# google/ffn

Hardware: NVIDIA H100
Metric: fov_steps_per_sec (higher is better)
Workload: dtype f16

## Files before the change

ffn_b200/_lib.py:

```python

from __future__ import annotations

import ctypes as C
import os

import numpy as np

HERE = os.path.dirname(os.path.abspath(__file__))
LIB_PATH = os.path.join(HERE, 'libffn_b200.so')

COMPUTE_FP16_TC = 0
COMPUTE_FP32 = 1
COMPUTE_FP16X2_TC = 2
IMAGE_U8 = 0
IMAGE_F32 = 1
ARRAY_SEED = 0
ARRAY_SEGMENTATION = 1
ARRAY_QPROB = 2
ARRAY_IMAGE = 3
MASK_MOVEMENT = 0
MASK_SEED = 1
SEED_POLICY_KINDS = {'peaks_2d': 0, 'fill_empty': 1, 'max_peaks': 2}

EXPORTS = [
    'ffn_last_error', 'ffn_engine_create', 'ffn_engine_destroy', 'ffn_engine_set_compute_mode', 'ffn_engine_set_chains', 'ffn_engine_set_grid',
    'ffn_engine_info', 'ffn_engine_profile', 'ffn_engine_trace', 'ffn_predict', 'ffn_canvas_create', 'ffn_canvas_destroy',
    'ffn_canvas_set_mask', 'ffn_canvas_segment_at', 'ffn_canvas_segment_all',
    'ffn_canvas_update_at', 'ffn_canvas_init_seed', 'ffn_canvas_read', 'ffn_canvas_write',
    'ffn_canvas_policy_state_size', 'ffn_canvas_policy_state_get', 'ffn_canvas_policy_state_set',
    'ffn_canvas_set_resume', 'ffn_canvas_trace', 'ffn_canvas_seed_peaks', 'ffn_canvas_seed_policy', 'ffn_canvas_set_max_id', 'ffn_canvas_get_counters', 'ffn_canvas_spec_stats', 'ffn_canvas_device_ptr',
    'ffn_canvas_add_id_offset', 'ffn_decision_points', 'ffn_reseg_eval', 'ffn_selftest_wgmma',
]


class ModelDesc(C.Structure):
  _fields_ = [('fov_zyx', C.c_int32 * 3), ('deltas_zyx', C.c_int32 * 3), ('depth', C.c_int32),
              ('features', C.c_int32)]


class Options(C.Structure):
  _fields_ = [('init_activation', C.c_float), ('pad_value', C.c_float),
              ('move_threshold', C.c_float), ('segment_threshold', C.c_float),
              ('disco_seed_threshold', C.c_float), ('policy_score_threshold', C.c_double),
              ('min_boundary_dist_zyx', C.c_int32 * 3), ('min_segment_size', C.c_int32)]


class SegStats(C.Structure):
  _fields_ = [('iters', C.c_int64), ('min_pos', C.c_int32 * 3), ('max_pos', C.c_int32 * 3),
              ('seed_got_too_weak', C.c_int32), ('queue_len', C.c_int32), ('finished', C.c_int32),
              ('reserved', C.c_int32)]


class Origin(C.Structure):
  _fields_ = [('id', C.c_int32), ('start_zyx', C.c_int32 * 3), ('iters', C.c_int64),
              ('walltime_sec', C.c_double)]


class Overlap(C.Structure):
  _fields_ = [('id', C.c_int32), ('other_id', C.c_int32), ('count', C.c_int64)]
# ... 32 lines not shown


_lib = None


def build_if_needed():
  from . import build as _build
  return _build.build()


def load() -> C.CDLL:
  global _lib
  if _lib is not None:
    return _lib
  if not os.path.exists(LIB_PATH):
    try:
      build_if_needed()
    except Exception as e:
      raise ImportError(
          'libffn_b200.so is missing and could not be built (%s). The FFN engine has no CPU '
          'fallback.' % e) from e
  lib = C.CDLL(LIB_PATH)
  p = C.c_void_p
  i32p = C.POINTER(C.c_int32)
  lib.ffn_last_error.restype = C.c_char_p
  lib.ffn_last_error.argtypes = []
  lib.ffn_engine_create.argtypes = [C.c_int, C.POINTER(ModelDesc), C.POINTER(C.c_void_p),
                                    C.POINTER(C.c_void_p), C.c_int, C.POINTER(p)]
  lib.ffn_engine_destroy.argtypes = [p]
  lib.ffn_engine_destroy.restype = None
  lib.ffn_engine_set_compute_mode.argtypes = [p, C.c_int]
  lib.ffn_engine_set_grid.argtypes = [p, C.c_int]
  lib.ffn_engine_set_chains.argtypes = [p, C.c_int]
  lib.ffn_engine_info.argtypes = [p, C.POINTER(C.c_int64)]
  lib.ffn_engine_profile.argtypes = [p, C.POINTER(C.c_int64), C.c_int]
  lib.ffn_engine_trace.argtypes = [p, C.POINTER(C.c_int64), C.c_int64, C.c_int]
  lib.ffn_predict.argtypes = [p, p, p, C.c_int, p]
  lib.ffn_canvas_create.argtypes = [p, p, C.c_int, i32p, C.c_float, C.c_float, C.POINTER(Options),
                                    C.c_int, C.POINTER(p)]
  lib.ffn_canvas_destroy.argtypes = [p]
  lib.ffn_canvas_destroy.restype = None
  lib.ffn_canvas_set_mask.argtypes = [p, C.c_int, p]
  lib.ffn_canvas_segment_at.argtypes = [p, i32p, C.c_int, C.c_int64, C.POINTER(SegStats)]
  lib.ffn_canvas_segment_all.argtypes = [p, p, C.c_int64, p, C.c_int64, C.POINTER(C.c_int64), p,
                                         C.c_int64, C.POINTER(C.c_int64), C.POINTER(Counters)]
  lib.ffn_canvas_update_at.argtypes = [p, i32p, p]
  lib.ffn_canvas_init_seed.argtypes = [p, i32p]
  lib.ffn_canvas_read.argtypes = [p, C.c_int, i32p, i32p, p]
  lib.ffn_canvas_write.argtypes = [p, C.c_int, i32p, i32p, p]
  lib.ffn_canvas_policy_state_size.argtypes = [p, C.POINTER(C.c_int64), C.POINTER(C.c_int64)]
  lib.ffn_canvas_policy_state_get.argtypes = [p, p, p, i32p]
  lib.ffn_canvas_policy_state_set.argtypes = [p, p, C.c_int64, p, C.c_int64, i32p]
  lib.ffn_canvas_set_resume.argtypes = [p, C.c_int64, i32p, i32p]
  lib.ffn_canvas_trace.argtypes = [p, C.c_int64, p, C.POINTER(C.c_int64)]
  lib.ffn_canvas_seed_peaks.argtypes = [p, C.POINTER(C.c_float), p, p, C.c_int64, C.POINTER(C.c_int64)]
  lib.ffn_canvas_seed_policy.argtypes = [p, C.POINTER(SeedPolicyDesc), p, p, C.c_int64, C.POINTER(C.c_int64)]
  lib.ffn_canvas_set_max_id.argtypes = [p, C.c_int64]
  lib.ffn_canvas_get_counters.argtypes = [p, C.POINTER(Counters)]
  lib.ffn_canvas_spec_stats.argtypes = [p, C.POINTER(C.c_int64)]
  lib.ffn_canvas_device_ptr.argtypes = [p, C.c_int, C.POINTER(p), C.POINTER(C.c_int64)]
  lib.ffn_canvas_add_id_offset.argtypes = [p, C.c_int32]
  lib.ffn_decision_points.argtypes = [C.c_int, C.POINTER(DecisionPointDesc), p, p, C.c_int64, C.POINTER(C.c_int64)]
  lib.ffn_reseg_eval.argtypes = [C.c_int, C.POINTER(ResegEvalDesc), p, p, p, p, p, p, C.c_int64, C.POINTER(C.c_int64)]
  lib.ffn_selftest_wgmma.argtypes = [C.c_int, C.POINTER(C.c_double), C.c_int]
  for name in EXPORTS:
    if name not in ('ffn_last_error', 'ffn_engine_destroy', 'ffn_canvas_destroy'):
# ... 17 lines not shown
```

ffn_b200/csrc/device_types.cuh:

```cuda
#pragma once

#include <cuda.h>
#include <cuda_fp16.h>
#include <cuda_runtime.h>
#include <stdint.h>

#include "../../include/ffn_b200.h"

namespace ffn {

constexpr int kThreads = 320;
constexpr int kLoadWarp = 8;
constexpr int kSigWarp = 9;
constexpr int kActStages = 3;
constexpr int kTileM = 128;
constexpr int kTileOut = 126;
constexpr int kStackN = 96;
constexpr int kFeat = 32;
constexpr int kAccRegs = 64 * kStackN / 128;
constexpr int kMaxConv = 32;
constexpr int kMaxChains = 4;
constexpr int kBufsPerChain = 6;
constexpr int kMaxBufs = kMaxChains * kBufsPerChain;
constexpr int kSplitShift = 10;
constexpr int kMaxTilesPerCta = 0xFFFF / kTileOut;
static_assert(kMaxChains >= 1 && kMaxChains <= 5, "chains");

struct Geom {
  int fz, fy, fx;
  int mz, my, mx;
  int dz, dy, dx;
  int nconv;
  int xp, pp;
  int nr;
  int nt;
  int halo;
  int guard;
  int rows_alloc;
  int V;
  float inv_pp, inv_xp;
};

struct Weights {
  const __half* w16;
  const __half* w16x2;
  const float* w32;
  const float* bias;
  const float* w_lom;
  float b_lom;
};

constexpr int kTraceEvents = 8, kTraceTiles = 2048, kTraceCta = 1;

constexpr unsigned kRowValid = 1, kRowX0 = 2, kRowXLast = 4;

struct Workspace {
  const uint8_t* row_flags;
  __half* act0_l;
  __half* act_l[2];
  float4* act0_f;
  float4* act_f[2];
  float4* res;
  unsigned* bar;
  int* abort_flag;
  long long* prof;
};

struct CanvasDev {
  const void* image;
  int image_is_u8;
  float mean, stddev;
  int* seg;
  uint8_t* qprob;
  const uint8_t* mask;
  const uint8_t* seed_mask;
  int sz, sy, sx;
  FfnOptions opt;
  float policy_th_f32;
  int q_cap;
  int traj_cap;
  int* trace;
  int trace_cap;
  int lat_dim[3], lat_off[3];
};

struct CanvasState;
struct ObjDev {
  float* seed;
  float* q_score;
  int* q_pos;
  unsigned* lattice;
  int* traj;
  CanvasState* st;
};

struct ChainDev {
  __half* act0_h;
  __half* act_h[2];
  float* seed_raw[2];
  float* logits;
  unsigned* count;
  unsigned* bar;
  float* res;
};

enum Phase : int {
  PH_IDLE = 0,
  PH_START_SEGMENT,
  PH_AFTER_CLEAR,
  PH_AFTER_STEP,
  PH_POP,
  PH_NEXT_SEED,
  PH_AFTER_COUNT,
  PH_AFTER_WRITE,
  PH_SEGMENT_DONE,
  PH_ALL_DONE,
  PH_FORCE_STEP,
  PH_FINISHED,
  PH_FREE,
};

struct CanvasState {
  int phase;
  int q_head, q_tail;
  unsigned epoch;
  int start[3];
  int cur[3];
  int have_cur;
  int min_pos[3], max_pos[3];
  long long iters;
  int dirty_lo[3], dirty_hi[3];
  long long seed_index;
  int spec;
  int fin_round;
  int reset_seed;
// ... 143 lines not shown
```

ffn_b200/csrc/engine.cu:

```cuda
#include <algorithm>
#include <cmath>
#include <cstdio>
#include <cstdlib>
#include <cstring>
#include <memory>
#include <string>
#include <vector>

#include "device_types.cuh"
#define FFN_KNS plain
#define FFN_PROFILE 0
#include "flood_kernel.cuh"
#undef FFN_KNS
#undef FFN_PROFILE
#define FFN_KNS profiled
#define FFN_PROFILE 1
#include "flood_kernel.cuh"
#undef FFN_KNS
#undef FFN_PROFILE
#include "seed_kernels.cuh"
#include "decision_kernels.cuh"
#include "reseg_kernels.cuh"
#include "selftest.cuh"

// ... 164 lines not shown
}

int launch(FfnEngine* e, FfnCanvas* c, int nchains, const Job& job) {
  KParams p{};
  p.g = e->g;
  p.w = e->w;
  p.ws = e->ws;
  if (!e->profiling) p.ws.prof = nullptr;
  if (c) p.cv = c->cv;
  p.nchains = nchains;
  for (int k = 0; k < kMaxChains; ++k) p.ch[k] = e->cws[k];
  for (int b = 0; b < kMaxBufs; ++b) {
    if (c && b < c->nbufs_alloc) p.ob[b] = c->ob[b];
    p.ob[b].st = c ? c->d_state + b : e->d_dummy_state + b;
  }
  p.sched = c ? c->d_sched : e->d_dummy_sched;
  p.ctl = e->d_ctl;
  p.round_flag = e->d_round_flag;
  p.snap = c ? c->d_snap : nullptr;
  std::memcpy(p.tmap, e->tmap, sizeof(p.tmap));
  p.use_tmap = e->use_tmap;
  p.job = job;
  {
    const char* env = std::getenv("FFN_B200_WATCHDOG_S");
    const long long secs = env ? std::atoll(env) : 60;
    p.job.watchdog_ns = (secs > 0 ? secs : 60) * 1000000000ll;
  }
  p.compute_mode = e->compute_mode;
  CUDA_OK(cudaMemsetAsync(e->ws.bar, 0, sizeof(unsigned), cudaStreamPerThread));
  CUDA_OK(cudaMemsetAsync(e->ws.abort_flag, 0, sizeof(int), cudaStreamPerThread));
  CUDA_OK(cudaMemsetAsync(e->d_ctl, 0, sizeof(Ctl), cudaStreamPerThread));
  CUDA_OK(cudaMemsetAsync(e->d_round_flag, 0, sizeof(unsigned), cudaStreamPerThread));
  for (int k = 0; k < kMaxChains; ++k) CUDA_OK(cudaMemsetAsync(e->cws[k].bar, 0, sizeof(unsigned), cudaStreamPerThread));
  void* args[] = {&p};
  CUDA_OK(cudaEventRecord(e->ev0, cudaStreamPerThread));
  CUDA_OK(cudaLaunchCooperativeKernel(flood_kernel(e), dim3(e->grid), dim3(kThreads), args, (size_t)e->smem_bytes,
                                      cudaStreamPerThread));
  CUDA_OK(cudaEventRecord(e->ev1, cudaStreamPerThread));
  CUDA_OK(cudaStreamSynchronize(cudaStreamPerThread));
  float ms = 0.f;
  CUDA_OK(cudaEventElapsedTime(&ms, e->ev0, e->ev1));
  e->last_kernel_seconds = ms * 1e-3;
  e->launches++;
  int abort_flag = 0;
  CUDA_OK(cudaMemcpy(&abort_flag, e->ws.abort_flag, sizeof(int), cudaMemcpyDeviceToHost));
  if (abort_flag != 0)
    return fail("device-side wait timed out (abort code " + std::to_string(abort_flag) +
                "): 1 = grid barrier, 2 = mbarrier, 3 = chain barrier, 4 = round flag, 5 = launch exceeded 60 s");
  return 0;
}

int pull_state(FfnCanvas* c) {
  CUDA_OK(cudaMemcpy(&c->h_state, c->d_state, sizeof(CanvasState), cudaMemcpyDeviceToHost));
  return 0;
}
int push_state(FfnCanvas* c) {
  CUDA_OK(cudaMemcpy(c->d_state, &c->h_state, sizeof(CanvasState), cudaMemcpyHostToDevice));
  return 0;
}

int alloc_buf(FfnCanvas* c, int k) {
  ObjDev& ch = c->ob[k];
  if (k > 0) {
    if (dev_alloc(&ch.seed, c->nvox, false)) return 1;
    fill_f32_kernel<<<c->eng->sm_count * 8, 256, 0, cudaStreamPerThread>>>(ch.seed, c->nvox, NAN);
    CUDA_OK(cudaGetLastError());
// ... 58 lines not shown

void pack_weights(const Geom& g, const float* const* w, std::vector<__half>& w16, std::vector<__half>& w16x2,
                  std::vector<float>& w32) {
  const int nconv = g.nconv;
  w16.assign(w16_layer_offset_halfs(nconv), __float2half(0.f));
  w16x2.assign(2 * w16_layer_offset_halfs(nconv), __float2half(0.f));
  w32.assign(w32_layer_offset_floats(nconv), 0.f);
  for (int l = 0; l < nconv; ++l) {
    const int cin = l == 0 ? 2 : 32;
    const int nch = l == 0 ? 2 : 4;
    const int cin_pad = l == 0 ? 4 : 32;
    __half* d16 = w16.data() + w16_layer_offset_halfs(l);
    __half* d16hi = w16x2.data() + 2 * w16_layer_offset_halfs(l);
    __half* d16lo = d16hi + (w16_layer_offset_halfs(l + 1) - w16_layer_offset_halfs(l));
    float* d32 = w32.data() + w32_layer_offset_floats(l);
    for (int tap = 0; tap < 27; ++tap)
      for (int ci = 0; ci < cin; ++ci)
        for (int co = 0; co < 32; ++co) {
          const float v = w[l][((size_t)tap * cin + ci) * 32 + co];
          {
            const int row = tap / 3, n = (tap % 3) * 32 + co;
            const size_t at = (((size_t)row * nch + ci / 8) * 12 + n / 8) * 64 + (n % 8) * 8 + (ci % 8);
            d16[at] = __float2half_rn(v);
            const float vs = v * (float)(1 << kSplitShift);
            const __half h = __float2half_rn(vs);
            d16hi[at] = h;
            d16lo[at] = __float2half_rn(vs - __half2float(h));
          }
          d32[((size_t)tap * cin_pad + ci) * 32 + co] = v;
        }
  }
}

int box_copy(FfnCanvas* c, int which, const int32_t lo[3], const int32_t sz[3], void* host, bool to_host) {
  const CanvasDev& cv = c->cv;
  for (int k = 0; k < 3; ++k) {
    const int dim = k == 0 ? cv.sz : k == 1 ? cv.sy : cv.sx;
    if (lo[k] < 0 || sz[k] <= 0 || lo[k] + sz[k] > dim) return fail("box out of canvas bounds");
  }
  size_t esz = 0;
  char* base = nullptr;
  switch (which) {
    case FFN_ARRAY_SEED: esz = 4; base = reinterpret_cast<char*>(c->ob[0].seed); break;
    case FFN_ARRAY_SEGMENTATION: esz = 4; base = reinterpret_cast<char*>(cv.seg); break;
    case FFN_ARRAY_QPROB:
      if (!cv.qprob) return fail("canvas was created without probability maps");
      esz = 1; base = reinterpret_cast<char*>(cv.qprob); break;
    default: return fail("unknown array id");
  }
  cudaMemcpy3DParms prm{};
  cudaPitchedPtr dev = make_cudaPitchedPtr(base, (size_t)cv.sx * esz, (size_t)cv.sx * esz, cv.sy);
  cudaPitchedPtr hst = make_cudaPitchedPtr(host, (size_t)sz[2] * esz, (size_t)sz[2] * esz, sz[1]);
  prm.extent = make_cudaExtent((size_t)sz[2] * esz, sz[1], sz[0]);
  if (to_host) {
    prm.srcPtr = dev;
    prm.srcPos = make_cudaPos((size_t)lo[2] * esz, lo[1], lo[0]);
    prm.dstPtr = hst;
    prm.kind = cudaMemcpyDeviceToHost;
  } else {
    prm.dstPtr = dev;
    prm.dstPos = make_cudaPos((size_t)lo[2] * esz, lo[1], lo[0]);
    prm.srcPtr = hst;
    prm.kind = cudaMemcpyHostToDevice;
  }
  CUDA_OK(cudaMemcpy3D(&prm));
  return 0;
// ... 69 lines not shown
  CUDA_OK(cudaMemcpy(d_wlom, weights_dhwio[g.nconv], 32 * sizeof(float), cudaMemcpyHostToDevice));
  e->w.w16 = d_w16;
  e->w.w32 = d_w32;
  e->w.bias = d_bias;
  e->w.w_lom = d_wlom;
  e->w.b_lom = biases[g.nconv][0];
  e->owned = {d_w16, d_w16x2, d_w32, d_bias, d_wlom};

  Workspace& ws = e->ws;
  const size_t ra = (size_t)g.rows_alloc;
  if (dev_alloc(&ws.act0_l, 2 * ra * 8)) return 1;
  if (dev_alloc(&ws.act_l[0], 4 * ra * 8)) return 1;
  if (dev_alloc(&ws.act_l[1], 4 * ra * 8)) return 1;
  if (dev_alloc(&ws.act0_f, ra)) return 1;
  if (dev_alloc(&ws.act_f[0], 8 * ra)) return 1;
  if (dev_alloc(&ws.act_f[1], 8 * ra)) return 1;
  if (dev_alloc(&ws.res, 8 * ra)) return 1;
  if (dev_alloc(&ws.bar, 1)) return 1;
  if (dev_alloc(&ws.abort_flag, 1)) return 1;
  if (dev_alloc(&ws.prof, 32 + kTraceEvents * kTraceTiles)) return 1;
  for (void* p : std::vector<void*>{ws.act0_l, ws.act_l[0], ws.act_l[1], ws.act0_f, ws.act_f[0], ws.act_f[1], ws.res,
                                    ws.bar, ws.abort_flag, ws.prof})
    e->owned.push_back(p);
  {
    std::vector<uint8_t> flags((size_t)g.nt * 64);
    for (int t = 0; t < g.nt; ++t)
      for (int i = 0; i < 64; ++i) flags[(size_t)t * 64 + i] = row_flags_byte(g, t, i / 8, i % 8);
    uint8_t* d_flags = nullptr;
    if (dev_alloc(&d_flags, flags.size())) return 1;
    e->owned.push_back(d_flags);
    CUDA_OK(cudaMemcpy(d_flags, flags.data(), flags.size(), cudaMemcpyHostToDevice));
    ws.row_flags = d_flags;
  }
  for (int k = 0; k < kMaxChains; ++k) {
    ChainDev& cw = e->cws[k];
    if (dev_alloc(&cw.act0_h, 2 * ra * 8)) return 1;
    if (dev_alloc(&cw.act_h[0], 4 * ra * 8)) return 1;
    if (dev_alloc(&cw.act_h[1], 4 * ra * 8)) return 1;
    if (dev_alloc(&cw.seed_raw[0], (size_t)g.nt * kTileM)) return 1;
    if (dev_alloc(&cw.seed_raw[1], (size_t)g.nt * kTileM)) return 1;
    if (dev_alloc(&cw.logits, (size_t)g.nt * kTileM)) return 1;
    if (dev_alloc(&cw.count, 4)) return 1;
    if (dev_alloc(&cw.bar, 1)) return 1;
    if (dev_alloc(&cw.res, (size_t)g.nt * kTileM * kFeat)) return 1;
    for (void* p : std::vector<void*>{cw.act0_h, cw.act_h[0], cw.act_h[1], cw.seed_raw[0], cw.seed_raw[1], cw.logits,
                                      cw.count, cw.bar, cw.res})
      e->owned.push_back(p);
  }
  {
    typedef CUresult (*EncodeFn)(CUtensorMap*, CUtensorMapDataType, cuuint32_t, void*, const cuuint64_t*, const cuuint64_t*,
                                 const cuuint32_t*, const cuuint32_t*, CUtensorMapInterleave, CUtensorMapSwizzle,
                                 CUtensorMapL2promotion, CUtensorMapFloatOOBfill);
    void* fn = nullptr;
    cudaDriverEntryPointQueryResult qres;
    bool ok = cudaGetDriverEntryPoint("cuTensorMapEncodeTiled", &fn, cudaEnableDefault, &qres) == cudaSuccess && fn &&
              qres == cudaDriverEntryPointSuccess;
    const int seg_rows = kTileOut + 2 * g.halo;
    for (int k = 0; ok && k < kMaxChains; ++k)
      for (int i = 0; ok && i < 3; ++i) {
        const cuuint32_t nch = i == 0 ? 2 : 4;
        void* base = i == 0 ? (void*)e->cws[k].act0_h : (void*)e->cws[k].act_h[i - 1];
        const cuuint64_t dims[4] = {8, (cuuint64_t)(g.rows_alloc - 2 * g.pp), 3, nch};
        const cuuint64_t strides[3] = {16, (cuuint64_t)g.pp * 16, (cuuint64_t)g.rows_alloc * 16};
        const cuuint32_t box[4] = {8, (cuuint32_t)seg_rows, 3, nch};
        const cuuint32_t estr[4] = {1, 1, 1, 1};
        ok = reinterpret_cast<EncodeFn>(fn)(&e->tmap[k][i], CU_TENSOR_MAP_DATA_TYPE_FLOAT16, 4, base, dims, strides, box, estr,
                                            CU_TENSOR_MAP_INTERLEAVE_NONE, CU_TENSOR_MAP_SWIZZLE_NONE,
                                            CU_TENSOR_MAP_L2_PROMOTION_L2_128B, CU_TENSOR_MAP_FLOAT_OOB_FILL_NONE) == CUDA_SUCCESS;
      }
    const char* env = std::getenv("FFN_B200_TMAP");
    e->use_tmap = (ok && env && std::atoi(env) != 0) ? 1 : 0;
  }
  if (dev_alloc(&e->d_ctl, 1)) return 1;
  if (dev_alloc(&e->d_round_flag, 1)) return 1;
  if (dev_alloc(&e->d_dummy_state, kMaxBufs)) return 1;
  if (dev_alloc(&e->d_dummy_sched, 1)) return 1;
  for (void* p : std::vector<void*>{e->d_ctl, e->d_round_flag, e->d_dummy_state, e->d_dummy_sched}) e->owned.push_back(p);
  *out = e.release();
  return 0;
}

void ffn_engine_destroy(FfnEngine* e) {
  if (!e || e->closing) return;
  if (e->live_canvases > 0) {
    e->closing = true;
    return;
  }
  engine_free(e);
}

int ffn_engine_set_grid(FfnEngine* e, int num_ctas) {
  if (!e) return fail("null engine");
  if (num_ctas <= 0) num_ctas = std::min(e->sm_count, e->g.nt);
  if (num_ctas > e->sm_count || num_ctas > e->g.nt) return fail("grid larger than the SM / tile count");
  if ((e->g.nt + num_ctas - 1) / num_ctas > kMaxTilesPerCta)
    return fail("grid too small: at most " + std::to_string(kMaxTilesPerCta) + " tiles per CTA");
  e->grid = num_ctas;
  return 0;
}

int ffn_engine_set_chains(FfnEngine* e, int max_chains) {
  if (!e) return fail("null engine");
  if (max_chains <= 0) max_chains = kMaxChains;
  if (max_chains > kMaxChains) return fail("at most " + std::to_string(kMaxChains) + " chains");
  e->max_chains = max_chains;
  return 0;
}

int ffn_engine_set_compute_mode(FfnEngine* e, int mode) {
  if (!e) return fail("null engine");
  if (mode != FFN_COMPUTE_FP16_TC && mode != FFN_COMPUTE_FP32 && mode != FFN_COMPUTE_FP16X2_TC)
    return fail("unknown compute mode");
  e->compute_mode = mode;
  return 0;
}

int ffn_engine_info(FfnEngine* e, int64_t info[8]) {
  if (!e || !info) return fail("null argument");
  info[0] = e->sm_count;
  info[1] = e->grid;
  info[2] = e->smem_bytes;
  info[3] = e->g.nt;
  info[4] = e->g.nr;
  info[5] = e->g.V;
  info[6] = e->launches;
  info[7] = (int64_t)(e->last_kernel_seconds * 1e9);
  return 0;
}

int ffn_engine_profile(FfnEngine* e, int64_t out[32], int reset) {
// ... 1113 lines not shown
```

ffn_b200/csrc/flood_kernel.cuh:

```cuda

#include <math_constants.h>

#include <utility>

#include "device_types.cuh"
#include "sm90.cuh"

namespace ffn {
namespace FFN_KNS {

struct Ctx {
  const KParams* p;
  int tid, warp, lane, cta, G;
  int t_begin, t_end;
  unsigned bar_target;
  unsigned ev0, ev1, ev2, ev3, ev4;
  unsigned round;
  unsigned long long t_start;
  unsigned char* smem;
  float* s_bias;
  uint64_t* mb_w;
  uint64_t* mb_full;
  uint64_t* mb_empty;
  uint64_t* mb_sig;
  unsigned load_cnt, epi_cnt;
  int* s_misc;
  int* s_round;
  float* s_xchg;
  CanvasState* s_state;
  Sched* s_sched;
  long long* prof;
#if FFN_PROFILE
  unsigned sig_cnt;
#endif
  uint32_t bits;
};

__device__ __forceinline__ uint32_t bit_get(const Ctx& c, int k) { return (c.bits >> k) & 1u; }
__device__ __forceinline__ void bit_flip(Ctx& c, int k) { c.bits ^= 1u << k; }
__device__ __forceinline__ void bit_set(Ctx& c, int k, bool v) { c.bits = (c.bits & ~(1u << k)) | ((v ? 1u : 0u) << k); }

__device__ __forceinline__ unsigned ev_get(const Ctx& c, int k) {
  return k == 0 ? c.ev0 : (k == 1 ? c.ev1 : (k == 2 ? c.ev2 : (k == 3 ? c.ev3 : c.ev4)));
}
__device__ __forceinline__ void ev_add(Ctx& c, int k, unsigned n) {
  if (k == 0) c.ev0 += n;
  else if (k == 1) c.ev1 += n;
  else if (k == 2) c.ev2 += n;
  else if (k == 3) c.ev3 += n;
  else c.ev4 += n;
}
__device__ __forceinline__ CanvasState* chain_state(const Ctx& c, int k) {
  return reinterpret_cast<CanvasState*>(reinterpret_cast<unsigned char*>(c.s_state) + k * kStateSlot);
}

__device__ __forceinline__ void chain_tiles(const Ctx& c, int k, int& tb, int& te) {
  const int nt = c.p->g.nt, base = nt / c.G, extra = nt % c.G;
  const int q = (c.cta + c.G - (k * extra) % c.G) % c.G;
  tb = q * base + min(q, extra);
  te = tb + base + (q < extra ? 1 : 0);
}

__device__ __forceinline__ bool aborted(const Ctx& c) {
  return sm90::ld_volatile_s32(c.p->ws.abort_flag) != 0;
}

#if FFN_PROFILE
__device__ __forceinline__ long long prof_now(const Ctx& c) { return c.prof ? clock64() : 0ll; }
__device__ __forceinline__ void prof_add(const Ctx& c, int slot, long long dt) {
  if (c.prof) c.prof[slot] += dt;
}
__device__ __forceinline__ void trace_ev(const Ctx& c, int ev, unsigned idx) {
  long long* trace = c.p->ws.prof;
  if (trace && c.cta == kTraceCta && idx < (unsigned)kTraceTiles) trace[32 + ev * kTraceTiles + idx] = clock64();
}
#else
__device__ __forceinline__ long long prof_now(const Ctx&) { return 0ll; }
__device__ __forceinline__ void prof_add(const Ctx&, int, long long) {}
__device__ __forceinline__ void trace_ev(const Ctx&, int, unsigned) {}
#endif

__device__ __forceinline__ void mbar_wait(const Ctx& c, uint64_t* bar, uint32_t parity) {
  unsigned spins = 0;
  long long t0 = 0;
  while (!sm90::mbar_try_wait(bar, parity)) {
    if ((++spins & 0x3FF) == 0) {
      if (aborted(c)) return;
      const long long now = clock64();
      if (t0 == 0) t0 = now;
      if (now - t0 > (1ll << 32)) {
        atomicExch(c.p->ws.abort_flag, 2);
        return;
      }
// ... 10 lines not shown
      const long long now = clock64();
      if (tw == 0) tw = now;
      if (now - tw > (1ll << 32)) {
        atomicExch(c.p->ws.abort_flag, code);
        break;
      }
    }
  }
}

__device__ __forceinline__ void grid_barrier(Ctx& c) {
  __syncthreads();
  c.bar_target += c.G;
  if (c.warp == kLoadWarp) {
    if (c.lane == 0) {
      const long long t0 = prof_now(c);
      sm90::red_release_add(c.p->ws.bar, 1u);
      spin_until(c, c.p->ws.bar, c.bar_target, 1);
      prof_add(c, 0, prof_now(c) - t0);
    }
    __syncwarp();
    asm volatile("bar.arrive 4, %0;" ::"n"(kThreads) : "memory");
  } else {
    asm volatile("bar.sync 4, %0;" ::"n"(kThreads) : "memory");
  }
}

__device__ __forceinline__ void chain_arrive_epi(Ctx& c, int k) {
  __syncwarp();
  if (c.lane == 0) sm90::mbar_arrive(&c.mb_sig[k]);
}
__device__ __forceinline__ void chain_signal(Ctx& c, int k, uint32_t parity) {
  mbar_wait(c, &c.mb_sig[k], parity);
  if (c.lane == 0) sm90::red_release_add(c.p->ch[k].bar, 1u);
  __syncwarp();
}
__device__ __forceinline__ void chain_wait(Ctx& c, int k, unsigned events) {
  if (c.lane == 0) {
    const long long t0 = prof_now(c);
    spin_until(c, c.p->ch[k].bar, (unsigned)c.G * (ev_get(c, k) + events), 3);
    prof_add(c, 14, prof_now(c) - t0);
  }
  __syncwarp();
}

__device__ __forceinline__ bool row_to_zyx(const Geom& g, int r, int& z, int& y, int& x) {
  if (r >= g.nr) return false;
  z = (int)(((float)r + 0.5f) * g.inv_pp);
  const int rem = r - z * g.pp;
  y = (int)(((float)rem + 0.5f) * g.inv_xp);
  x = rem - y * g.xp;
  return y < g.fy && x < g.fx;
}

__device__ __forceinline__ bool disco_active(const KParams& p, int k, unsigned parity) {
  if (!(p.cv.opt.disco_seed_threshold >= 0.f)) return false;
  const unsigned cnt = __ldcg(p.ch[k].count + 2 * parity);
  return (double)cnt / (double)p.g.V > (double)p.cv.opt.disco_seed_threshold;
}

__device__ __forceinline__ float merged_row(const KParams& p, int k, unsigned parity, int r, bool disco) {
  float l = __ldcg(p.ch[k].logits + r);
  if (disco) {
    const float o = __ldcg(p.ch[k].seed_raw[parity] + r);
    if (o < 0.f && l > o) l = o;
  }
  return l;
}

__device__ __forceinline__ void stage_fov(Ctx& c, int k, int b, int pz, int py, int px, int batch_idx) {
  const KParams& p = *c.p;
  const Geom& g = p.g;
  const ChainDev& ch = p.ch[k];
  const bool predict = p.job.mode == MODE_PREDICT;
  const unsigned par = c.round & 1u;
// ... 302 lines not shown
}

template <bool X2>
__device__ __forceinline__ int tc_epilogue_any(Ctx& c, int k, int layer, int tile, const EpiBase& e, unsigned flags,
                                               const float (&d)[kAccRegs]) {
  if (layer == c.p->g.nconv - 1) return tc_epilogue<EPI_LAST, X2>(c, k, layer, tile, e, flags, d);
  if (!(layer & 1)) return tc_epilogue<EPI_A, X2>(c, k, layer, tile, e, flags, d);
  if (layer == 1) return tc_epilogue<EPI_B_FIRST, X2>(c, k, layer, tile, e, flags, d);
  return tc_epilogue<EPI_B, X2>(c, k, layer, tile, e, flags, d);
}

__device__ __forceinline__ void publish_counts(Ctx& c, int k, int hit) {
  hit = __reduce_add_sync(0xffffffffu, hit);
  if (c.lane == 0 && hit) atomicAdd(&c.s_misc[k], hit);
  asm volatile("bar.sync 5, 256;" ::: "memory");
  if (c.tid == 0 && c.s_misc[k]) {
    const unsigned packed = (unsigned)c.s_misc[k];
    unsigned* cnt = c.p->ch[k].count + 2 * (c.round & 1u);
    if (packed & 0xffffu) atomicAdd(cnt, packed & 0xffffu);
    if (packed >> 16) atomicAdd(cnt + 1, packed >> 16);
  }
}

__device__ __forceinline__ void layers_pipelined(Ctx& c, unsigned mask) {
  const KParams& p = *c.p;
  const Geom& g = p.g;
  unsigned char* act_smem = c.smem + 2 * 27 * 4 * 512;
  const int seg_rows = kTileOut + 2 * g.halo;
  const int stage_bytes = 3 * 4 * seg_rows * 16;
  const int nconv = g.nconv;
  if (c.tid == 0) prof_add(c, 11, -prof_now(c));

  if (c.warp == kLoadWarp) {
    for (int layer = 0; layer < nconv; ++layer) {
      const int nch = layer == 0 ? 2 : 4;
      const unsigned n0 = c.load_cnt;
      bool weights_pending = true;
      for (int k = 0; k < kMaxChains; ++k) {
        if (!((mask >> k) & 1u)) continue;
        const ChainDev& ch = p.ch[k];
        const __half* in = layer == 0 ? ch.act0_h : ch.act_h[(layer - 1) & 1];
        chain_wait(c, k, (unsigned)layer + 1u);
        if (c.lane == 0) trace_ev(c, 0, c.load_cnt);
        sm90::fence_proxy_async_global();
        int tb, te;
        chain_tiles(c, k, tb, te);
        for (int tile = tb; tile < te; ++tile) {
          const int s = c.load_cnt % kActStages;
          mbar_wait(c, &c.mb_empty[s], ((c.load_cnt / kActStages) & 1u) ^ 1u);
          if (weights_pending && c.load_cnt - n0 == (unsigned)(kActStages - 1)) {
            weights_pending = false;
            if (sm90::elect_one()) tc_issue_weight_load(c, (layer + 1 == nconv) ? 0 : layer + 1);
            __syncwarp();
          }
          const int r0 = tile * kTileOut;
          unsigned char* dst = act_smem + (size_t)s * stage_bytes;
          if (sm90::elect_one()) {
            sm90::mbar_expect_tx(&c.mb_full[s], (uint32_t)(3 * nch * seg_rows * 16));
            if (p.use_tmap) {
              sm90::tma_load_4d(dst, &p.tmap[k][layer == 0 ? 0 : 1 + ((layer - 1) & 1)], 0, g.guard + r0 - g.halo - g.pp, 0, 0,
                                &c.mb_full[s]);
            } else {
              for (int cc = 0; cc < nch; ++cc)
                for (int dzi = 0; dzi < 3; ++dzi)
                  sm90::bulk_g2s(dst + (size_t)(cc * 3 + dzi) * seg_rows * 16,
                                 in + ((size_t)cc * g.rows_alloc + g.guard + r0 + (dzi - 1) * g.pp - g.halo) * 8,
                                 (uint32_t)seg_rows * 16, &c.mb_full[s]);
            }
          }
          __syncwarp();
          if (c.lane == 0) trace_ev(c, 1, c.load_cnt);
          ++c.load_cnt;
        }
      }
      if (weights_pending) {
// ... 1343 lines not shown
  }
}

__device__ __forceinline__ void commit_write(Ctx& c, int b) {
  const KParams& p = *c.p;
  const CanvasState* st = p.ob[b].st;
  int lo[3], hi[3];
  load3(st->box_lo, lo);
  load3(st->box_hi, hi);
  const int nz = hi[0] - lo[0], ny = hi[1] - lo[1], nx = hi[2] - lo[2];
  const long long lines = (long long)nz * ny;
  const int sid = __ldcg(&st->cur_sid);
  for (long long l = (long long)c.cta * (kThreads / 32) + c.warp; l < lines; l += (long long)c.G * (kThreads / 32)) {
    const int z = lo[0] + (int)(l / ny), y = lo[1] + (int)(l % ny);
    const size_t base = cv_index(p.cv, z, y, lo[2]);
    for (int x = c.lane; x < nx; x += 32) {
      const float s = __ldcg(p.ob[b].seed + base + x);
      if (!(s >= p.cv.opt.segment_threshold)) continue;
      if (__ldcg(p.cv.seg + base + x) > 0) continue;
      p.cv.seg[base + x] = sid;
      if (p.cv.qprob) p.cv.qprob[base + x] = quantize_prob(s);
    }
  }
}

template <bool kSplit>
__device__ __forceinline__ void run_layers(Ctx& c, unsigned mask) {
  const KParams& p = *c.p;
  if (!kSplit && p.compute_mode == FFN_COMPUTE_FP16_TC) {
    __syncthreads();
    if (c.tid == 0) {
#pragma unroll
      for (int k = 0; k < kMaxChains; ++k)
        if ((mask >> k) & 1u) sm90::red_release_add(p.ch[k].bar, 1u);
    }
    layers_pipelined(c, mask);
  } else {
    layers_blocking<kSplit>(c);
  }
}

template <bool kSplit>
__global__ void __launch_bounds__(kThreads, 1) ffn_flood_kernel(const __grid_constant__ KParams p) {
  extern __shared__ __align__(1024) unsigned char smem_raw[];
  Ctx c;
  c.p = &p;
  c.tid = threadIdx.x;
  c.warp = __shfl_sync(0xffffffffu, (int)(threadIdx.x >> 5), 0);
  c.lane = threadIdx.x & 31;
  c.cta = blockIdx.x;
  c.G = gridDim.x;
  c.t_begin = (int)(((long long)c.cta * p.g.nt) / c.G);
  c.t_end = (int)(((long long)(c.cta + 1) * p.g.nt) / c.G);
  c.bar_target = 0;
  c.ev0 = c.ev1 = c.ev2 = c.ev3 = c.ev4 = 0;
  c.round = 0;
  c.t_start = sm90::globaltimer_ns();
  c.smem = smem_raw;
  const SmemLayout L = smem_layout(p.g);
  c.s_bias = reinterpret_cast<float*>(smem_raw + L.bias);
  c.mb_w = reinterpret_cast<uint64_t*>(smem_raw + L.bars);
  c.mb_full = c.mb_w + 2;
  c.mb_empty = c.mb_full + kActStages;
  c.mb_sig = c.mb_empty + kActStages;
  c.load_cnt = c.epi_cnt = 0;
  c.s_misc = reinterpret_cast<int*>(smem_raw + L.bars + kOffMisc);
  c.s_round = reinterpret_cast<int*>(smem_raw + L.bars + kOffRound);
// ... 187 lines not shown
```

include/ffn_b200.h:

```cpp
#ifndef FFN_B200_H_
#define FFN_B200_H_

#include <stdint.h>

#ifdef __cplusplus
extern "C" {
#endif

typedef struct FfnEngine FfnEngine;
typedef struct FfnCanvas FfnCanvas;

enum {
  FFN_COMPUTE_FP16_TC = 0,
  FFN_COMPUTE_FP32 = 1,
  FFN_COMPUTE_FP16X2_TC = 2
};

enum { FFN_IMAGE_U8 = 0, FFN_IMAGE_F32 = 1 };

enum { FFN_ARRAY_SEED = 0, FFN_ARRAY_SEGMENTATION = 1, FFN_ARRAY_QPROB = 2, FFN_ARRAY_IMAGE = 3 };

enum { FFN_MASK_MOVEMENT = 0, FFN_MASK_SEED = 1 };

typedef struct {
// ... 34 lines not shown
typedef struct {
  int32_t id;
  int32_t other_id;
  int64_t count;
} FfnOverlap;

typedef struct {
  int64_t inference_calls;
  int64_t segment_at_calls;
  int64_t seeds_examined;
  int64_t skip_threshold;
  int64_t skip_invalid_pos;
  int64_t skip_restricted_pos;
  int64_t seed_got_too_weak;
  int64_t voxels_segmented;
  int64_t voxels_overlapping;
  int64_t invalid_weak;
  int64_t invalid_small;
  int64_t invalid_other;
  int64_t segments;
  int64_t max_id;
  double device_seconds;
  int64_t kernel_launches;
} FfnCounters;

const char* ffn_last_error(void);

int ffn_engine_create(int device, const FfnModelDesc* model, const float* const* weights_dhwio,
                      const float* const* biases, int compute_mode, FfnEngine** out);
void ffn_engine_destroy(FfnEngine* engine);
int ffn_engine_set_compute_mode(FfnEngine* engine, int compute_mode);
int ffn_engine_set_chains(FfnEngine* engine, int max_chains);
int ffn_engine_set_grid(FfnEngine* engine, int num_ctas);
int ffn_engine_info(FfnEngine* engine, int64_t info[8]);

int ffn_engine_profile(FfnEngine* engine, int64_t out[32], int reset);
int ffn_engine_trace(FfnEngine* engine, int64_t* out, int64_t n, int reset);

int ffn_predict(FfnEngine* engine, const float* seed, const float* image, int batch,
                float* logits_out);

int ffn_canvas_create(FfnEngine* engine, const void* image, int image_dtype,
                      const int32_t shape_zyx[3], float image_mean, float image_stddev,
                      const FfnOptions* options, int keep_probability_maps, FfnCanvas** out);
void ffn_canvas_destroy(FfnCanvas* canvas);
int ffn_canvas_set_mask(FfnCanvas* canvas, int which, const uint8_t* mask);

int ffn_canvas_segment_at(FfnCanvas* canvas, const int32_t start_zyx[3], int reset,
                          int64_t max_steps, FfnSegStats* out);

int ffn_canvas_segment_all(FfnCanvas* canvas, const int32_t* seeds_zyx, int64_t n_seeds,
                           FfnOrigin* origins_out, int64_t origins_cap, int64_t* n_origins,
                           FfnOverlap* overlaps_out, int64_t overlaps_cap, int64_t* n_overlaps,
                           FfnCounters* counters_out);

int ffn_canvas_update_at(FfnCanvas* canvas, const int32_t pos_zyx[3], float* pred_out);

int ffn_canvas_init_seed(FfnCanvas* canvas, const int32_t pos_zyx[3]);

int ffn_canvas_read(FfnCanvas* canvas, int which, const int32_t lo_zyx[3],
                    const int32_t size_zyx[3], void* dst);
int ffn_canvas_write(FfnCanvas* canvas, int which, const int32_t lo_zyx[3],
                     const int32_t size_zyx[3], const void* src);

int ffn_canvas_policy_state_size(FfnCanvas* canvas, int64_t* queue_len, int64_t* done_len);
int ffn_canvas_policy_state_get(FfnCanvas* canvas, double* queue_szyx, int32_t* done_zyx,
// ... 81 lines not shown
```

Measured before the change: 6367.

## Replace grid-wide chain barrier with per-CTA progress counters and neighbour waits

Each CTA now publishes its own progress counter per chain, and the load warp waits only on the CTAs whose tile ranges overlap its halo, using a host-computed neighbour table, instead of a barrier counting signals from the whole grid. The aim is to stop a CTA from stalling on slow, unrelated CTAs between conv layers so layers can overlap across the grid. In exchange it adds more polling loads, a neighbour-table upload whenever the grid changes, and a correctness risk if the halo reasoning behind the table is wrong.

```diff
diff --git a/ffn_b200/_lib.py b/ffn_b200/_lib.py
--- a/ffn_b200/_lib.py
+++ b/ffn_b200/_lib.py
@@ -24,7 +24,7 @@
 
 EXPORTS = [
     'ffn_last_error', 'ffn_engine_create', 'ffn_engine_destroy', 'ffn_engine_set_compute_mode', 'ffn_engine_set_chains', 'ffn_engine_set_grid',
-    'ffn_engine_info', 'ffn_engine_profile', 'ffn_engine_trace', 'ffn_predict', 'ffn_canvas_create', 'ffn_canvas_destroy',
+    'ffn_chain_neighbours', 'ffn_engine_info', 'ffn_engine_profile', 'ffn_engine_trace', 'ffn_predict', 'ffn_canvas_create', 'ffn_canvas_destroy',
     'ffn_canvas_set_mask', 'ffn_canvas_segment_at', 'ffn_canvas_segment_all',
     'ffn_canvas_update_at', 'ffn_canvas_init_seed', 'ffn_canvas_read', 'ffn_canvas_write',
     'ffn_canvas_policy_state_size', 'ffn_canvas_policy_state_get', 'ffn_canvas_policy_state_set',
@@ -123,6 +123,7 @@
   lib.ffn_engine_set_compute_mode.argtypes = [p, C.c_int]
   lib.ffn_engine_set_grid.argtypes = [p, C.c_int]
   lib.ffn_engine_set_chains.argtypes = [p, C.c_int]
+  lib.ffn_chain_neighbours.argtypes = [C.POINTER(ModelDesc), C.c_int, C.c_int, i32p, i32p]
   lib.ffn_engine_info.argtypes = [p, C.POINTER(C.c_int64)]
   lib.ffn_engine_profile.argtypes = [p, C.POINTER(C.c_int64), C.c_int]
   lib.ffn_engine_trace.argtypes = [p, C.POINTER(C.c_int64), C.c_int64, C.c_int]
diff --git a/ffn_b200/csrc/device_types.cuh b/ffn_b200/csrc/device_types.cuh
--- a/ffn_b200/csrc/device_types.cuh
+++ b/ffn_b200/csrc/device_types.cuh
@@ -41,6 +41,18 @@
   float inv_pp, inv_xp;
 };
 
+__host__ __device__ inline void chain_tiles(int nt, int G, int k, int cta, int& tb, int& te) {
+  const int base = nt / G, extra = nt % G;
+  const int q = (cta + G - (k * extra) % G) % G;
+  tb = q * base + (q < extra ? q : extra);
+  te = tb + base + (q < extra ? 1 : 0);
+}
+
+constexpr int kMaxNeighbours = 32;
+constexpr int kMaxNeighbourGrid = 255;
+constexpr int kProgStride = 8;
+static_assert(kMaxChains <= 4, "the neighbour table packs 16 bits per chain into 64");
+
 struct Weights {
   const __half* w16;
   const __half* w16x2;
@@ -62,6 +74,7 @@
   float4* act_f[2];
   float4* res;
   unsigned* bar;
+  const uint64_t* nbr;
   int* abort_flag;
   long long* prof;
 };
@@ -101,6 +114,7 @@
   float* logits;
   unsigned* count;
   unsigned* bar;
+  unsigned* prog;
   float* res;
 };
 
diff --git a/ffn_b200/csrc/engine.cu b/ffn_b200/csrc/engine.cu
--- a/ffn_b200/csrc/engine.cu
+++ b/ffn_b200/csrc/engine.cu
@@ -220,6 +220,7 @@
   CUDA_OK(cudaMemsetAsync(e->d_ctl, 0, sizeof(Ctl), cudaStreamPerThread));
   CUDA_OK(cudaMemsetAsync(e->d_round_flag, 0, sizeof(unsigned), cudaStreamPerThread));
   for (int k = 0; k < kMaxChains; ++k) CUDA_OK(cudaMemsetAsync(e->cws[k].bar, 0, sizeof(unsigned), cudaStreamPerThread));
+  CUDA_OK(cudaMemsetAsync(e->cws[0].prog, 0, (size_t)kMaxChains * e->sm_count * kProgStride * sizeof(unsigned), cudaStreamPerThread));
   void* args[] = {&p};
   CUDA_OK(cudaEventRecord(e->ev0, cudaStreamPerThread));
   CUDA_OK(cudaLaunchCooperativeKernel(flood_kernel(e), dim3(e->grid), dim3(kThreads), args, (size_t)e->smem_bytes,
@@ -344,6 +345,48 @@
   }
 }
 
+void chain_neighbours(const Geom& g, int G, int k, int32_t* first, int32_t* count) {
+  const int base = g.nt / G, extra = g.nt % G, rot = (k * extra) % G;
+  auto slot_of = [&](int t) { return t < extra * (base + 1) ? t / (base + 1) : extra + (t - extra * (base + 1)) / base; };
+  std::vector<int> rlo(G), rhi(G);
+  for (int q = 0; q < G; ++q) {
+    int tb, te;
+    ffn::chain_tiles(g.nt, G, k, (q + rot) % G, tb, te);
+    const int lo = tb * kTileOut - g.pp - g.halo, hi = te * kTileOut + g.pp + g.halo;
+    rlo[q] = slot_of(std::max(lo, 0) / kTileOut);
+    rhi[q] = slot_of(std::min((hi - 1) / kTileOut, g.nt - 1));
+  }
+  std::vector<int> lo(G), hi(G);
+  bool whole = false;
+  for (int q = 0; q < G; ++q) {
+    lo[q] = rlo[q];
+    hi[q] = rhi[q];
+    for (int i = 0; i < G; ++i)
+      if (rlo[i] <= q && q <= rhi[i]) {
+        lo[q] = std::min(lo[q], i);
+        hi[q] = std::max(hi[q], i);
+      }
+    whole |= hi[q] - lo[q] + 1 > kMaxNeighbours;
+  }
+  for (int q = 0; q < G; ++q) {
+    const int cta = (q + rot) % G;
+    first[cta] = whole ? 0 : (lo[q] + rot) % G;
+    count[cta] = whole ? G : hi[q] - lo[q] + 1;
+  }
+}
+
+int upload_neighbours(FfnEngine* e) {
+  const int G = e->grid;
+  std::vector<uint64_t> packed(G, 0);
+  std::vector<int32_t> first(G), count(G);
+  for (int k = 0; k < kMaxChains; ++k) {
+    chain_neighbours(e->g, G, k, first.data(), count.data());
+    for (int j = 0; j < G; ++j) packed[j] |= (uint64_t)((uint32_t)first[j] | (uint32_t)count[j] << 8) << (16 * k);
+  }
+  CUDA_OK(cudaMemcpy(const_cast<uint64_t*>(e->ws.nbr), packed.data(), G * sizeof(uint64_t), cudaMemcpyHostToDevice));
+  return 0;
+}
+
 int box_copy(FfnCanvas* c, int which, const int32_t lo[3], const int32_t sz[3], void* host, bool to_host) {
   const CanvasDev& cv = c->cv;
   for (int k = 0; k < 3; ++k) {
@@ -479,6 +522,17 @@
     CUDA_OK(cudaMemcpy(d_flags, flags.data(), flags.size(), cudaMemcpyHostToDevice));
     ws.row_flags = d_flags;
   }
+  if (e->sm_count > kMaxNeighbourGrid) return fail("more SMs than the neighbour table of the chain waits holds");
+  {
+    uint64_t* d_nbr = nullptr;
+    unsigned* d_prog = nullptr;
+    if (dev_alloc(&d_nbr, (size_t)e->sm_count)) return 1;
+    if (dev_alloc(&d_prog, (size_t)kMaxChains * e->sm_count * kProgStride)) return 1;
+    e->owned.push_back(d_nbr);
+    e->owned.push_back(d_prog);
+    ws.nbr = d_nbr;
+    for (int k = 0; k < kMaxChains; ++k) e->cws[k].prog = d_prog + (size_t)k * e->sm_count * kProgStride;
+  }
   for (int k = 0; k < kMaxChains; ++k) {
     ChainDev& cw = e->cws[k];
     if (dev_alloc(&cw.act0_h, 2 * ra * 8)) return 1;
@@ -523,6 +577,7 @@
   if (dev_alloc(&e->d_dummy_state, kMaxBufs)) return 1;
   if (dev_alloc(&e->d_dummy_sched, 1)) return 1;
   for (void* p : std::vector<void*>{e->d_ctl, e->d_round_flag, e->d_dummy_state, e->d_dummy_sched}) e->owned.push_back(p);
+  if (upload_neighbours(e.get())) return 1;
   *out = e.release();
   return 0;
 }
@@ -542,7 +597,19 @@
   if (num_ctas > e->sm_count || num_ctas > e->g.nt) return fail("grid larger than the SM / tile count");
   if ((e->g.nt + num_ctas - 1) / num_ctas > kMaxTilesPerCta)
     return fail("grid too small: at most " + std::to_string(kMaxTilesPerCta) + " tiles per CTA");
+  if (set_device(e)) return 1;
   e->grid = num_ctas;
+  return upload_neighbours(e);
+}
+
+int ffn_chain_neighbours(const FfnModelDesc* model, int num_ctas, int chain, int32_t* first, int32_t* count) {
+  if (!model || !first || !count) return fail("null argument");
+  for (int k = 0; k < 3; ++k)
+    if (model->fov_zyx[k] < 3 || model->fov_zyx[k] % 2 == 0) return fail("fov sizes must be odd and >= 3");
+  const Geom g = make_geom(*model);
+  if (num_ctas < 1 || num_ctas > g.nt || num_ctas > kMaxNeighbourGrid) return fail("grid outside [1, min(tiles, 255)]");
+  if (chain < 0 || chain >= kMaxChains) return fail("bad chain index");
+  chain_neighbours(g, num_ctas, chain, first, count);
   return 0;
 }
 
diff --git a/ffn_b200/csrc/flood_kernel.cuh b/ffn_b200/csrc/flood_kernel.cuh
--- a/ffn_b200/csrc/flood_kernel.cuh
+++ b/ffn_b200/csrc/flood_kernel.cuh
@@ -55,10 +55,7 @@
 }
 
 __device__ __forceinline__ void chain_tiles(const Ctx& c, int k, int& tb, int& te) {
-  const int nt = c.p->g.nt, base = nt / c.G, extra = nt % c.G;
-  const int q = (c.cta + c.G - (k * extra) % c.G) % c.G;
-  tb = q * base + min(q, extra);
-  te = tb + base + (q < extra ? 1 : 0);
+  ffn::chain_tiles(c.p->g.nt, c.G, k, c.cta, tb, te);
 }
 
 __device__ __forceinline__ bool aborted(const Ctx& c) {
@@ -135,15 +132,43 @@
 }
 __device__ __forceinline__ void chain_signal(Ctx& c, int k, uint32_t parity) {
   mbar_wait(c, &c.mb_sig[k], parity);
-  if (c.lane == 0) sm90::red_release_add(c.p->ch[k].bar, 1u);
+  if (c.lane == 0) sm90::red_release_add(c.p->ch[k].prog + c.cta * kProgStride, 1u);
   __syncwarp();
 }
-__device__ __forceinline__ void chain_wait(Ctx& c, int k, unsigned events) {
+__device__ __forceinline__ void chain_wait_staged(Ctx& c, int k) {
   if (c.lane == 0) {
     const long long t0 = prof_now(c);
-    spin_until(c, c.p->ch[k].bar, (unsigned)c.G * (ev_get(c, k) + events), 3);
+    spin_until(c, c.p->ch[k].bar, (unsigned)c.G * (ev_get(c, k) / (unsigned)c.p->g.nconv + 1u), 3);
     prof_add(c, 14, prof_now(c) - t0);
   }
+  __syncwarp();
+}
+__device__ __forceinline__ void chain_wait_neighbours(Ctx& c, int k, unsigned events, uint32_t nb) {
+  const long long t0 = prof_now(c);
+  const int first = (int)(nb & 0xFFu), count = (int)((nb >> 8) & 0xFFu);
+  const unsigned target = ev_get(c, k) + events;
+  const unsigned* prog = c.p->ch[k].prog;
+  unsigned spins = 0;
+  long long tw = 0;
+  for (;;) {
+    bool done = true;
+    for (int i = c.lane; i < count; i += 32) {
+      const int j = first + i < c.G ? first + i : first + i - c.G;
+      done &= (int)(sm90::ld_acquire_u32(prog + j * kProgStride) - target) >= 0;
+    }
+    if (__all_sync(0xffffffffu, done)) break;
+    if ((++spins & 0xFF) == 0) {
+      const bool stop = aborted(c);
+      const long long now = clock64();
+      if (tw == 0) tw = now;
+      const bool late = now - tw > (1ll << 32);
+      if (__any_sync(0xffffffffu, stop || late)) {
+        if (late && !stop) atomicExch(c.p->ws.abort_flag, 3);
+        break;
+      }
+    }
+  }
+  if (c.lane == 0) prof_add(c, 14, prof_now(c) - t0);
   __syncwarp();
 }
 
@@ -512,6 +537,7 @@
   if (c.tid == 0) prof_add(c, 11, -prof_now(c));
 
   if (c.warp == kLoadWarp) {
+    const uint64_t nbr = __ldg(p.ws.nbr + c.cta);
     for (int layer = 0; layer < nconv; ++layer) {
       const int nch = layer == 0 ? 2 : 4;
       const unsigned n0 = c.load_cnt;
@@ -520,7 +546,11 @@
         if (!((mask >> k) & 1u)) continue;
         const ChainDev& ch = p.ch[k];
         const __half* in = layer == 0 ? ch.act0_h : ch.act_h[(layer - 1) & 1];
-        chain_wait(c, k, (unsigned)layer + 1u);
+        if (layer == 0) {
+          chain_wait_staged(c, k);
+        } else {
+          chain_wait_neighbours(c, k, (unsigned)layer + 1u, (uint32_t)(nbr >> (16 * k)) & 0xFFFFu);
+        }
         if (c.lane == 0) trace_ev(c, 0, c.load_cnt);
         sm90::fence_proxy_async_global();
         int tb, te;
@@ -1930,7 +1960,10 @@
     if (c.tid == 0) {
 #pragma unroll
       for (int k = 0; k < kMaxChains; ++k)
-        if ((mask >> k) & 1u) sm90::red_release_add(p.ch[k].bar, 1u);
+        if ((mask >> k) & 1u) {
+          sm90::red_release_add(p.ch[k].bar, 1u);
+          sm90::red_release_add(p.ch[k].prog + c.cta * kProgStride, 1u);
+        }
     }
     layers_pipelined(c, mask);
   } else {
diff --git a/include/ffn_b200.h b/include/ffn_b200.h
--- a/include/ffn_b200.h
+++ b/include/ffn_b200.h
@@ -90,6 +90,7 @@
 int ffn_engine_set_compute_mode(FfnEngine* engine, int compute_mode);
 int ffn_engine_set_chains(FfnEngine* engine, int max_chains);
 int ffn_engine_set_grid(FfnEngine* engine, int num_ctas);
+int ffn_chain_neighbours(const FfnModelDesc* model, int num_ctas, int chain, int32_t* first, int32_t* count);
 int ffn_engine_info(FfnEngine* engine, int64_t info[8]);
 
 int ffn_engine_profile(FfnEngine* engine, int64_t out[32], int reset);
```

Result: faster. 6480, median of 6 (+1.8%).
